# gwenzhang/GGA

Measured on AMD Instinct MI355X. Metric: kitti_frames_per_sec_gga_train_step, higher is better.
Workload: dtype f32 tensors; products on 2 x f16 operand planes (block-scaled), f32 accumulate - measured no less accurate than fp32 kernels: per convolution 0.7 x (dense) / 0.7-1.2 x (sparse) the RMS error of an fp32 FMA chain vs float64, whole-step losses over 8 seeds <= 2.5e-5 from float64 (fp32 CPU step: <= 1.6

## Files before the change

gga_amd/_lib.py:

```python
import ctypes as C
import os
import subprocess

_HERE = os.path.dirname(os.path.abspath(__file__))
LIB_PATH = os.path.join(_HERE, 'libgga_hip.so')
ABI_VERSION = 35

_lib = None

vp, i32, i64, f32, sz = C.c_void_p, C.c_int, C.c_int64, C.c_float, C.c_size_t
I3 = C.POINTER(C.c_int32 * 3)


class VoxelParams(C.Structure):
    _fields_ = [('voxel_size', C.c_float * 3), ('pc_range', C.c_float * 6),
                ('max_points', C.c_int32), ('max_voxels', C.c_int32)]


class PfnParams(C.Structure):
    _fields_ = [('voxel_size', C.c_float * 3), ('offsets', C.c_float * 3), ('eps', C.c_float),
                ('momentum', C.c_float), ('training', C.c_int32), ('in_features', C.c_int32),
                ('channels', C.c_int32)]


# ... 52 lines not shown
    'gga_hard_voxelize_workspace_bytes': (sz, [i32, i64]),
    'gga_hard_voxelize_batch': (i32, [vp, i32, C.POINTER(C.c_int64), i32, C.POINTER(VoxelParams),
                                       vp, vp, vp, vp, vp, sz, vp]),
    'gga_hard_voxelize_prepared': (i32, [vp, i32, C.POINTER(C.c_int64), vp, i32, C.POINTER(VoxelParams),
                                          vp, vp, vp, vp, vp, sz, vp]),
    'gga_dynamic_voxelize': (i32, [vp, i32, C.POINTER(C.c_int64), vp, i32, C.POINTER(VoxelParams), vp, vp, vp]),
    'gga_dynamic_voxel_map_workspace_bytes': (sz, [i64]),
    'gga_dynamic_voxel_map': (i32, [vp, vp, i32, i64, i32, i32, i32, i32, vp, vp, vp, vp, vp, vp, sz, vp]),
    'gga_dynamic_scatter_chunk': (i32, []),
    'gga_dynamic_scatter_workspace_bytes': (sz, [i64, i32]),
    'gga_dynamic_scatter_fwd': (i32, [vp, i32, i64, vp, vp, vp, vp, i64, i32, vp, vp, vp, sz, vp]),
    'gga_dynamic_scatter_bwd': (i32, [vp, i32, i64, vp, vp, vp, i64, i32, vp, vp]),
    'gga_dynamic_pfn_workspace_bytes': (sz, [i64]),
    'gga_dynamic_pfn_fwd': (i32, [vp, vp, i64, vp, vp, vp, vp, i64, C.POINTER(PfnParams)] + [vp] * 10 + [sz, vp]),
    'gga_dynamic_pfn_bwd': (i32, [vp, vp, i64, vp, i64, C.POINTER(PfnParams)] + [vp] * 11 + [sz, vp]),
    'gga_points_prepare_workspace_bytes': (sz, [i32, i64, i64]),
    'gga_points_prepare_batch': (i32, [vp, C.POINTER(C.c_int64), vp, C.POINTER(C.c_int64), vp, C.POINTER(C.c_int64),
                                        i32, i32, C.c_double, vp, C.POINTER(C.c_uint64), vp, vp, vp, sz, vp]),
    'gga_voxel_mean': (i32, [vp, vp, i64, i32, i32, i32, vp, vp]),
    'gga_pfn_workspace_bytes': (sz, [i64]),
    'gga_pfn_fwd': (i32, [vp, vp, vp, i64, vp, i32, C.POINTER(PfnParams), vp, vp, vp, vp, vp, vp, vp, vp, vp, sz, vp]),
    'gga_pfn_bwd': (i32, [vp, vp, vp, i64, vp, i32, C.POINTER(PfnParams), vp, vp, vp, vp, vp, vp, vp, vp, vp, vp, sz, vp]),
    'gga_pillar_scatter_map_bytes': (sz, [i32, i32, i32]),
    'gga_pillar_scatter_fwd': (i32, [vp, vp, i64, vp, i32, i32, i32, i32, i32, i32, vp, vp, vp]),
    'gga_pillar_scatter_bwd': (i32, [vp, vp, i64, vp, i32, i32, i32, i32, i32, vp, vp]),
    'gga_pillar_conv_map': (i32, [vp, i64, vp, i32, i32, i32, i32, i32, i32, i32, i32, i32, vp, vp]),
    'gga_sparse_index_bytes': (sz, [i64]),
    'gga_sparse_build_index': (i32, [vp, i64, i32, i32, i32, i32, vp, sz, vp]),
    'gga_sparse_out_index_bytes': (sz, [i64, i32]),
    'gga_sparse_out_sites_workspace_bytes': (sz, [i64, i32]),
    'gga_sparse_conv_out_sites': (i32, [vp, i64, i32, I3, I3, I3, I3, I3, vp, i64, vp, vp, sz, vp, sz, vp]),
    'gga_sparse_rulebook': (i32, [vp, i64, vp, i64, i32, I3, I3, I3, I3, I3, vp, i64, vp, i64, vp, vp, vp]),
    'gga_sparse_rowmask': (i32, [vp, i64, i32, vp, vp]),
    'gga_sparse_mask_order_workspace_bytes': (sz, [i64]),
    'gga_sparse_morton_order_workspace_bytes': (sz, [i64]),
    'gga_sparse_morton_order': (i32, [vp, i64, i32, i32, vp, vp, sz, vp]),
    'gga_sparse_mask_order': (i32, [vp, i64, i32, vp, vp, sz, vp]),
    'gga_sparse_split_weight_bytes': (sz, [i32, i32, i32]),
    'gga_sparse_conv_wgrad_workspace_bytes': (sz, [i64, i32, i32, i32]),
    'gga_dense_wgrad3x3_workspace_bytes': (sz, [i32, i32, i32, i32, i32]),
    'gga_sparse_pack_weight_planes': (i32, [vp, i32, i32, i32, i32, i32, vp, vp, vp]),
    'gga_sparse_conv_apply_stats': (i32, [vp, vp, vp, vp, vp, i64, i32, i32, i32, i32, vp, i64, i32, vp, vp, vp, vp]),
    'gga_sparse_conv_apply_tiles': (i64, [i64]),
    'gga_sparse_conv_apply_bn_bwd': (i32, [vp, vp, vp, vp, vp, i64, i32, i32, i32, i32, vp, i64, i32, vp, vp, vp, vp, i64, vp, vp, vp, vp, vp]),
    'gga_sparse_bev_nhwc_fwd': (i32, [vp, vp, i64, i32, i32, i32, i32, i32, vp, vp]),
    'gga_sparse_bev_nhwc_bwd': (i32, [vp, vp, i64, i32, i32, i32, i32, i32, vp, vp]),
    'gga_sparse_halo_tile_rows': (i64, []),
    'gga_sparse_halo_build': (i32, [vp, vp, i64, i64, i32, i32, vp, vp, vp, vp]),
    'gga_sparse_conv_apply_halo': (i32, [vp, vp, vp, vp, i32, vp, vp, i64, i64, i32, i32, i32, i32, vp, i64, i32, vp, vp, vp, vp, i64, vp, vp, vp, vp, vp]),
    'gga_sparse_conv_wgrad_planes': (i32, [vp, i64, vp, i64, vp, i64, i32, i32, i32, vp, i32, vp, vp, vp, sz, vp]),
    'gga_deconv_stream_tiles': (i64, [i64, i32, i32]),
    'gga_deconv_stream_fwd': (i32, [vp, vp, vp, vp, i32, i32, i32, i32, i32, i32, vp, vp, vp]),
    'gga_deconv_stream_bwd': (i32, [vp, vp, vp, vp, i32, i32, i32, i32, i32, i32, vp, vp]),
    'gga_absmax_bits': (i32, [vp, i64, i32, i64, vp, vp]),
    'gga_dense_conv3x3_pack_planes': (i32, [vp, i64, i64, i64, i64, i32, i32, i32, i32, vp, vp, vp]),
    'gga_dense_conv3x3_levels': (i32, [i32, vp, vp, vp, vp, i32, i32, i32, vp, i64, i32, vp, vp, vp, i32, i32, vp, vp]),
    'gga_dense_conv3x3_bn_bwd_pays': (i32, [i32, i32, i32, i32]),
    'gga_dense_conv3x3_bn_bwd_pays_planes': (i32, [i32, i32, i32, i32, i32]),
    'gga_dense_conv3x3_bn_bwd': (i32, [vp, vp, i32, i32, i32, i32, i32, vp, i64, i32, vp, i32, vp, vp, vp, i64, vp, vp, vp, vp, vp]),
    'gga_absmax_table_blocks': (i64, [i64]),
    'gga_absmax_table': (i32, [vp, i32, i64, vp, i32, vp]),
    'gga_pack_weights_table': (i32, [vp, i32, i64, i32, vp]),
    'gga_dense_wgrad3x3_block_amax': (i32, [vp, vp, i32, i32, i32, i32, i32, vp, i64, i64, i64, i64, i32, i32, vp, i32, vp, i32, vp, sz, vp]),
    'gga_dense_conv3x3_tile_rows': (i32, [i32, i32, i32, i32, i32]),
    'gga_dense_conv3x3_stat_rows': (i64, [i32, i32, i32, i32, i32, i32]),
    'gga_bn_relu_workspace_bytes': (sz, [i64, i32]),
    'gga_bn_relu_mask_bytes': (sz, [i64, i32]),
    'gga_bn_relu_fwd': (i32, [vp, vp, vp, vp, vp, vp, i64, i32, f32, f32, i32, i32, vp, i64, vp, vp, vp, i32, vp, vp, sz, vp]),
    'gga_bn_relu_bwd': (i32, [vp, i64, vp, vp, vp, vp, i64, i32, i32, i32, vp, vp, vp, vp, vp, vp, sz, vp]),
    'gga_column_sums': (i32, [vp, i64, i32, vp, vp, sz, vp]),
    'gga_bn_relu_bwd_partials': (i32, [vp, i64, vp, vp, vp, i64, i32, i32, vp, i32, vp, vp, vp, vp, vp, sz, vp]),
    'gga_gn_relu_workspace_bytes': (sz, [i32, i32]),
    'gga_gn_relu_fwd': (i32, [vp, vp, vp, i32, i64, i32, i32, f32, i32, vp, vp, vp, vp, vp, sz, vp]),
    'gga_gn_relu_bwd': (i32, [vp, vp, vp, vp, vp, i32, i64, i32, i32, i32, vp, vp, vp, vp, vp, sz, vp]),
    'gga_bn_stats': (i32, [vp, vp, vp, vp, vp, i64, i32, f32, f32, i32, vp, vp, vp, i32, i32, i32, vp, sz, vp]),
    'gga_head_conv3x3_fwd': (i32, [vp, i64, vp, vp, vp, i32, i32, i32, i32, i32, vp, vp]),
    'gga_head_conv3x3_fwd_tiles': (i32, [vp, i64, vp, vp, vp, i32, i32, i32, i32, i32, vp, vp, vp]),
    'gga_head_cell_tiles_count': (i64, [i32, i32, i32]),
    'gga_head_cell_tiles': (i32, [vp, i32, i32, i32, i32, vp, vp]),
    'gga_head_conv3x3_workspace_bytes': (sz, [i32]),
    'gga_head_conv3x3_wgrad': (i32, [vp, i64, vp, vp, i32, i32, i32, i32, i32, vp, vp, vp, sz, vp]),
    'gga_head_tail_bwd': (i32, [vp, vp, i64, vp, vp, vp, vp, i32, i32, i32, i32, i32, vp, i64, vp, vp, vp, vp, sz, vp]),
    'gga_head_tile_activity': (i32, [vp, i32, i32, i32, i32, vp, vp]),
    'gga_head_branch_bwd_workspace_bytes': (sz, [i32, i32, i32, i32]),
    'gga_head_branch_bwd': (i32, [vp, vp, i64, vp, vp, vp, vp, i32, i32, i32, i32, i32, vp, vp, vp, i64, vp, vp, vp, i32, vp, sz, vp]),
    'gga_heatmap_splat': (i32, [vp, i32, i32, i32, vp, i32, vp, vp, i32, vp]),
    'gga_focal_loss_workspace_bytes': (sz, [i64, i32]),
    'gga_focal_loss_fwd': (i32, [C.POINTER(TaskTable), f32, f32, f32, vp, sz, vp]),
    'gga_focal_loss_bwd': (i32, [C.POINTER(TaskTable), f32, f32, f32, vp]),
    'gga_gather_pred_fwd': (i32, [C.POINTER(TaskTable), i32, i32, i32, i32, vp]),
    'gga_gather_pred_bwd': (i32, [C.POINTER(TaskTable), i32, i32, i32, i32, vp]),
    'gga_box_losses_workspace_bytes': (sz, [i32, i32, i32]),
    'gga_box_losses_fwd': (i32, [C.POINTER(TaskTable), C.POINTER(LossParams), vp, sz, vp]),
    'gga_box_losses_bwd': (i32, [C.POINTER(TaskTable), i32, i32, vp]),
    'gga_box_iou_rotated': (i32, [vp, i32, vp, i32, i32, i32, vp, vp]),
    'gga_nms_rotated_workspace_bytes': (sz, [i32]),
    'gga_nms_rotated_sorted': (i32, [vp, i32, f32, i32, vp, vp, vp, sz, vp]),
    'gga_circle_nms_sorted': (i32, [vp, i32, C.c_double, i32, vp, vp, vp, sz, vp]),
    'gga_region_grow_workspace_bytes': (sz, [i64, i32]),
    'gga_region_grow': (i32, [vp, i64, i32, vp, vp, vp, i32, C.c_double, i32, vp, vp, sz, vp]),
    'gga_points_in_convex_polyhedra': (i32, [vp, i64, i32, vp, vp, i32, i32, vp, vp]),
    'gga_plane_inliers': (i32, [vp, i64, i32, vp, i32, C.c_double, vp, vp, vp]),
    'gga_image_box_match': (i32, [vp, vp, vp, vp, i32, i64, i32, vp, vp, vp, vp, vp]),
    'gga_kitti_eval_overlaps': (i32, [vp, vp, i64, vp, vp, i64, i32, i32, i32, i32, vp, vp, i64, vp]),
    'gga_kitti_eval_stats_workspace_bytes': (sz, [i32, i32, i32]),
    'gga_kitti_eval_stats': (i32, [vp, i32, vp, i64, vp, vp, vp, vp, i64, vp, i64, vp, i64, vp, vp, i32, vp, vp, i32, i32, i32, i32, i32,
# ... 69 lines not shown
```

gga_amd/pillar_conv.py:

```python
import torch
from torch import nn

from . import _lib
from . import functional as F
from ._lib import check


class PillarSupport:
    __slots__ = ('feats', 'coors', 'num_valid')

    def __init__(self, feats, coors, num_valid):
        self.feats, self.coors, self.num_valid = feats, coors, num_valid


def eligible(conv, canvas):
    sup = getattr(canvas, 'pillar_support', None)
    return (sup is not None and type(conv) is nn.Conv2d and conv.bias is None and conv.groups == 1
            and tuple(conv.dilation) == (1, 1) and conv.padding_mode == 'zeros' and not isinstance(conv.padding, str)
            and canvas.is_cuda and canvas.dtype == torch.float32 and torch.is_grad_enabled()
            and (sup.feats.requires_grad or conv.weight.requires_grad)
            and conv.in_channels <= 128 and conv.out_channels <= 128 and conv.in_channels % 4 == 0
            and canvas.is_contiguous(memory_format=torch.channels_last))


class _PillarConv2d(torch.autograd.Function):
    @staticmethod
    def forward(ctx, feats, weight, canvas, coors, num_valid, stride, padding):
        from . import strided_conv
        kh, kw = weight.shape[2:]
        if (strided_conv.ENABLED and kh == kw and stride[0] == stride[1] and padding[0] == padding[1] and stride[0] > 1
                and kh <= 5 and weight.shape[0] % 4 == 0):
            B, Ci, ny, nx = canvas.shape
            bk = strided_conv.book(B, ny, nx, kh, stride[0], padding[0], canvas.device)
            y, stats = strided_conv._apply(strided_conv._rows(canvas), bk.fwd, bk.fwd_mask, bk.fwd_perm,
                                           weight.detach().permute(2, 3, 1, 0).reshape(kh * kw, Ci, -1), bk.n_out,
                                           strided_conv._amax(feats.detach().contiguous()), want_stats=True)
            y = y.view(B, bk.Ho, bk.Wo, -1).permute(0, 3, 1, 2)
        else:
            y = torch.conv2d(canvas, weight, None, stride, padding)
            stats = torch.empty(0, dtype=torch.float64, device=y.device)
        ctx.save_for_backward(feats, weight, coors, num_valid)
        ctx.geom = (tuple(canvas.shape), stride, padding)
        ctx.mark_non_differentiable(stats)
        ctx.set_materialize_grads(False)
        return y, stats

    @staticmethod
    def backward(ctx, gy, _gstats=None):
        from .sparse import _Rulebook, _conv_apply, _pack_weight, conv_wgrad
        feats, w, coors, num_valid = ctx.saved_tensors
        (B, Ci, ny, nx), (sh, sw), (ph, pw) = ctx.geom
        Co, _, kh, kw = w.shape
        kvol, m = kh * kw, feats.shape[0]
        gy = gy.contiguous(memory_format=torch.channels_last)
        rows = gy.permute(0, 2, 3, 1).reshape(-1, Co)
        feats = feats.contiguous()
        L = _lib.lib()
        nbr = torch.empty((kvol, m), dtype=torch.int32, device=gy.device)
        check(L.gga_pillar_conv_map(F._p(coors), m, F._p(num_valid), B, ny, nx, kh, kw, sh, sw, ph, pw, F._p(nbr),
                                    F._stream()), 'gga_pillar_conv_map')
        gx = gw = None
        if ctx.needs_input_grad[0]:
            rb = _Rulebook(nbr)
            wk = w.permute(2, 3, 0, 1).reshape(kvol, Co, Ci).contiguous()
            gx = torch.empty_like(feats)
            _conv_apply(rows, rb, _pack_weight(wk, kvol, Co, Ci, 0), m, kvol, Co, Ci, 0, gx)
        if ctx.needs_input_grad[1]:
            g = torch.empty((kvol, Co, Ci), dtype=torch.float32, device=gy.device)
            conv_wgrad(rows, feats, nbr, m, kvol, Co, Ci, g)
            gw = g.view(kh, kw, Co, Ci).permute(2, 3, 0, 1)
        return gx, gw, None, None, None, None, None


def pillar_conv2d(canvas, conv):
    sup = canvas.pillar_support
    coors = sup.coors if sup.coors.dtype == torch.int32 else sup.coors.int()
    y, stats = _PillarConv2d.apply(sup.feats, conv.weight, canvas.detach(), coors.contiguous(), sup.num_valid,
                                   tuple(conv.stride), tuple(conv.padding))
    if stats.numel():
        F.attach_bn_partials(y, stats)
    return y
```

gga_amd/strided_conv.py:

```python
import ctypes as C
import os

import torch
from torch import nn

from . import _lib
from . import functional as F
from ._lib import check

ENABLED = True
STREAM = os.environ.get('GGA_DECONV_STREAM', '1') != '0'
STREAM_OFF = set()
_BOOKS = {}


class _Book:

    def __init__(self, B, H, W, k, s, p, device):
        Ho, Wo = (H + 2 * p - k) // s + 1, (W + 2 * p - k) // s + 1
        self.Ho, self.Wo, self.kvol = Ho, Wo, k * k
        self.n_in, self.n_out = B * H * W, B * Ho * Wo
        self._geom = (B, H, W, k, s, p, device)

    def __getattr__(self, name):
        side = name.split('_')[0]
        if side not in ('fwd', 'bwd') or name not in (side, side + '_mask', side + '_perm'):
            raise AttributeError(name)
        with torch.no_grad():
            m = self._map(side)
            mask, perm = self._order(m)
        self.__dict__.update({side: m, side + '_mask': mask, side + '_perm': perm})
        return self.__dict__[name]

    def _map(self, side):
        B, H, W, k, s, p, device = self._geom
        Ho, Wo = self.Ho, self.Wo
        b = torch.arange(B, device=device).view(B, 1, 1)
        oy, ox = torch.arange(Ho, device=device).view(1, Ho, 1), torch.arange(Wo, device=device).view(1, 1, Wo)
        iy_, ix_ = torch.arange(H, device=device).view(1, H, 1), torch.arange(W, device=device).view(1, 1, W)
        rows = []
        for ky in range(k):
            for kx in range(k):
                if side == 'fwd':
                    iy, ix = oy * s + ky - p, ox * s + kx - p
                    ok = (iy >= 0) & (iy < H) & (ix >= 0) & (ix < W)
                    rows.append(torch.where(ok, b * (H * W) + iy * W + ix, -1).reshape(-1))
                else:
                    ny, nx = iy_ + p - ky, ix_ + p - kx
                    ok = (ny >= 0) & (nx >= 0) & (ny % s == 0) & (nx % s == 0) & (ny // s < Ho) & (nx // s < Wo)
                    rows.append(torch.where(ok, b * (Ho * Wo) + (ny // s) * Wo + nx // s, -1).reshape(-1))
        return torch.stack(rows).int().contiguous()

    @staticmethod
    def _order(m):
        kvol, n = m.shape
        if kvol > 32:
            return None, None
        mask = torch.empty(n, dtype=torch.int32, device=m.device)
        check(_lib.lib().gga_sparse_rowmask(F._p(m), n, kvol, F._p(mask), F._stream()), 'gga_sparse_rowmask')
        if bool((mask == mask[0]).all()):
            return mask, None
        from .sparse import mask_order
        return mask, mask_order(mask, kvol)


# ... 32 lines not shown
            from . import dense_conv
            if dense_conv.RANGE_GUARD.armed:
                dense_conv.RANGE_GUARD.record(w_kio.detach())
    else:
        x_amax = w_amax = None
    y = torch.empty((n_rows, cout), dtype=torch.float32, device=x_rows.device)
    tiles = int(L.gga_sparse_conv_apply_tiles(n_rows)) if want_stats else 0
    parts = []
    for c0 in range(0, cout, 128):
        c1 = min(c0 + 128, cout)
        if bank:
            from . import weight_bank
            wp, w_amax = weight_bank.gather_operand(w_kio, planes, c0, c1)
        else:
            wp = torch.empty(L.gga_sparse_split_weight_bytes(kvol, cin, c1 - c0) // 2, dtype=torch.int16, device=y.device)
            check(L.gga_sparse_pack_weight_planes(F._p(w_kio[:, :, c0:c1].contiguous()), kvol, cin, c1 - c0, 0, planes, F._p(w_amax),
                                                  F._p(wp), F._stream()), 'gga_sparse_pack_weight_planes')
        st = torch.empty((tiles, 2, c1 - c0), dtype=torch.float64, device=y.device) if want_stats else None
        check(L.gga_sparse_conv_apply_stats(F._p(x_rows), F._p(m), F._p(wp), F._p(perm), F._p(mask), n_rows, kvol, cin,
                                            c1 - c0, 0, y.data_ptr() + 4 * c0, cout, planes, F._p(x_amax), F._p(w_amax),
                                            F._p(st), F._stream()), 'gga_sparse_conv_apply_stats')
        if want_stats:
            parts.append(st)
    if want_stats:
        return y, (parts[0] if len(parts) == 1 else torch.cat(parts, dim=2))
    return y


def _wgrad(x_rows, g_rows, m, n_rows, x_amax=None, g_amax=None):
    planes = _planes()
    if planes == 2:
        x_amax = _amax(x_rows) if x_amax is None else x_amax
        g_amax = _amax(g_rows) if g_amax is None else g_amax
    else:
        x_amax = g_amax = None
    L = _lib.lib()
    kvol, cin, cout = m.shape[0], x_rows.shape[1], g_rows.shape[1]
    gw = torch.empty((kvol, cin, cout), dtype=torch.float32, device=x_rows.device)
    for i0 in range(0, cin, 128):
        i1 = min(i0 + 128, cin)
        for o0 in range(0, cout, 128):
            o1 = min(o0 + 128, cout)
            whole = i1 - i0 == cin and o1 - o0 == cout
            part = gw if whole else torch.empty((kvol, i1 - i0, o1 - o0), dtype=torch.float32, device=gw.device)
            ws = F._workspace('sp_wgrad', L.gga_sparse_conv_wgrad_workspace_bytes(n_rows, kvol, i1 - i0, o1 - o0), gw.device)
            check(L.gga_sparse_conv_wgrad_planes(x_rows.data_ptr() + 4 * i0, cin, g_rows.data_ptr() + 4 * o0, cout, F._p(m),
                                                 n_rows, kvol, i1 - i0, o1 - o0, F._p(part), planes, F._p(x_amax), F._p(g_amax),
                                                 F._p(ws), ws.numel(), F._stream()), 'gga_sparse_conv_wgrad_planes')
            if not whole:
                gw[:, i0:i1, o0:o1] = part
    return gw


class _StridedConv(torch.autograd.Function):

    @staticmethod
    def forward(ctx, x, weight, k, s, p):
        B, cin, H, W = x.shape
        bk = book(B, H, W, k, s, p, x.device)
        w = weight.detach()
        x_amax = _amax(x)
        y, stats = _apply(_rows(x), bk.fwd, bk.fwd_mask, bk.fwd_perm, w.permute(2, 3, 1, 0), bk.n_out, x_amax, want_stats=True, bank=True)
        ctx.save_for_backward(x, weight)
        ctx.geom, ctx.amax = (k, s, p), (x_amax, None)
        ctx.mark_non_differentiable(stats)
        ctx.set_materialize_grads(False)
        return y.view(B, bk.Ho, bk.Wo, -1).permute(0, 3, 1, 2), stats

    @staticmethod
    def backward(ctx, gy, _gstats=None):
        x, weight = ctx.saved_tensors
        k, s, p = ctx.geom
        B, cin, H, W = x.shape
        cout = weight.shape[0]
        bk = book(B, H, W, k, s, p, x.device)
        gy = gy.contiguous(memory_format=torch.channels_last)
        g_rows = _rows(gy)
        gx = gw = None
        x_amax, w_amax = ctx.amax if _planes() == 2 else (None, None)
        g_amax = _amax(gy)
        if ctx.needs_input_grad[0]:
            w = weight.detach()
            gx = _apply(g_rows, bk.bwd, bk.bwd_mask, bk.bwd_perm, w.permute(2, 3, 0, 1), bk.n_in, g_amax, bank=True)
            gx = gx.view(B, H, W, cin).permute(0, 3, 1, 2)
        if ctx.needs_input_grad[1]:
            gw = _wgrad(_rows(x), g_rows, bk.fwd, bk.n_out, x_amax, g_amax).view(k, k, cin, cout).permute(3, 2, 0, 1)
        return gx, gw, None, None, None


def _stream_form(cin, cout, s, backward):
    if not STREAM or _planes() != 2 or cin not in (64, 128, 256) or cout % 128 or not 1 <= s <= 4:
        return False
    form = (s, 'bwd' if backward else 'fwd')
    return form not in STREAM_OFF and (not backward or cout in (128, 256, 512))


def _block_pointers(ops):
    return (C.c_void_p * len(ops))(*[op.data_ptr() for op in ops])


def _stream_fwd(x, weight, s, x_amax, want_stats=True):
    from . import dense_conv, weight_bank
    L = _lib.lib()
    B, cin, H, W = x.shape
    cout = weight.shape[1]
    w_kio = weight.detach().permute(2, 3, 0, 1)
    if dense_conv.RANGE_GUARD.armed:
        dense_conv.RANGE_GUARD.record(w_kio)
    ops = [weight_bank.gather_operand(w_kio, 2, c0, c0 + 128) for c0 in range(0, cout, 128)]
    x_amax = _amax(x) if x_amax is None else x_amax
    y = torch.empty((B, H * s, W * s, cout), dtype=torch.float32, device=x.device)
    tiles = int(L.gga_deconv_stream_tiles(B * H * W, cin, s))
    stats = torch.empty((tiles, 2, cout), dtype=torch.float64, device=x.device) if want_stats else None
    check(L.gga_deconv_stream_fwd(F._p(_rows(x)), _block_pointers([op for op, _ in ops]), F._p(x_amax), F._p(ops[0][1]), B, H, W,
                                  cin, cout, s, F._p(y), F._p(stats), F._stream()), 'gga_deconv_stream_fwd')
# ... 93 lines not shown
```

include/gga_hip.h:

```cpp
#ifndef GGA_HIP_H_
#define GGA_HIP_H_

#include <stddef.h>
#include <stdint.h>

#ifdef __cplusplus
extern "C" {
#endif

typedef enum {
    GGA_OK = 0,
    GGA_ERR_INVALID_ARG = -1,
    GGA_ERR_WORKSPACE = -2,
    GGA_ERR_LAUNCH = -3
} gga_status;

const char* gga_last_error(void);
int gga_abi_version(void);

enum {
    GGA_TIME_SCATTER_FWD = 0,
    GGA_TIME_DENSE_CONV = 1,
    GGA_TIME_SPARSE_CONV = 2,
    GGA_TIME_SPARSE_WGRAD = 3,
// ... 140 lines not shown
int64_t gga_dense_conv3x3_stat_rows(int B, int H, int W, int cout, int planes, int n_slices);
int gga_dense_conv3x3_tile_rows(int B, int H, int W, int cout, int planes);

int gga_absmax_bits(const float* x, int64_t rows, int width, int64_t row_stride, uint32_t* out_bits, void* stream);
typedef struct {
    const float* src;
    uint16_t* dst;
    const uint32_t* amax;
    int64_t s_k0, s_k1, s_c, s_col;
    int64_t first;
    int32_t kw, kvol, n_c, n_col, c0, col0, n_in, co, layout, reverse;
} GgaPackEntry;
typedef struct {
    const float* src;
    uint32_t* slot;
    int64_t n;
    int64_t first_block;
} GgaAmaxEntry;
int64_t gga_absmax_table_blocks(int64_t n);
int gga_absmax_table(const GgaAmaxEntry* table_device, int n_entries, int64_t n_blocks, uint32_t* slots, int n_slots, void* stream);
int gga_pack_weights_table(const GgaPackEntry* table_device, int n_entries, int64_t total, int planes, void* stream);
int gga_sparse_pack_weight_planes(const float* weight, int kvol, int cin, int cout, int transpose, int planes,
                                  const uint32_t* amax_weight, void* packed, void* stream);
int64_t gga_sparse_conv_apply_tiles(int64_t n_rows);
int gga_sparse_conv_apply_stats(const float* x, const int32_t* map, const void* split_weight, const int32_t* perm,
                                const uint32_t* rowmask, int64_t n_rows, int kvol, int cin, int cout, int flip, float* y,
                                int64_t y_row_stride, int planes, const uint32_t* amax_x, const uint32_t* amax_weight,
                                double* stats, void* stream);
int gga_sparse_conv_apply_bn_bwd(const float* x, const int32_t* map, const void* split_weight, const int32_t* perm,
                                 const uint32_t* rowmask, int64_t n_rows, int kvol, int cin, int cout, int flip, float* y,
                                 int64_t y_row_stride, int planes, const uint32_t* amax_x, const uint32_t* amax_weight,
                                 double* stats, const float* bn_x, int64_t bn_x_row_stride, const float* bn_gamma,
                                 const float* bn_beta, const float* bn_mean, const float* bn_invstd, void* stream);
int64_t gga_sparse_halo_tile_rows(void);
int gga_sparse_halo_build(const int32_t* nbr, const int32_t* tile_rows, int64_t n_rows, int64_t n_tiles, int kvol,
                          int halo_capacity, int32_t* halo_rows, int32_t* halo_counts, uint16_t* local_map, void* stream);
int gga_sparse_conv_apply_halo(const float* x, const void* split_weight, const int32_t* tile_rows,
                               const int32_t* halo_counts, int halo_capacity, const int32_t* halo_rows,
                               const uint16_t* local_map, int64_t n_rows, int64_t n_tiles, int kvol, int cin, int cout, int flip,
                               float* y, int64_t y_row_stride, int planes, const uint32_t* amax_x, const uint32_t* amax_weight,
                               double* stats, const float* bn_x, int64_t bn_x_row_stride, const float* bn_gamma,
                               const float* bn_beta, const float* bn_mean, const float* bn_invstd, void* stream);
size_t gga_sparse_conv_wgrad_workspace_bytes(int64_t n_rows, int kvol, int cin, int cout);
int gga_sparse_conv_wgrad_planes(const float* x, int64_t x_row_stride, const float* grad_out, int64_t grad_out_row_stride,
                                 const int32_t* nbr, int64_t n_rows, int kvol, int cin, int cout, float* grad_weight,
                                 int planes, const uint32_t* amax_x, const uint32_t* amax_grad_out, void* workspace,
                                 size_t workspace_bytes, void* stream);
int64_t gga_deconv_stream_tiles(int64_t n_pixels, int cin, int s);
int gga_deconv_stream_fwd(const float* x, const void* const* weight_blocks, const uint32_t* amax_x,
                          const uint32_t* amax_weight, int B, int h, int w, int cin, int cout, int s, float* y, double* stats,
                          void* stream);
int gga_deconv_stream_bwd(const float* gy, const void* const* weight_blocks, const uint32_t* amax_gy,
                          const uint32_t* amax_weight, int B, int h, int w, int cin, int cout, int s, float* gx, void* stream);
int gga_dense_conv3x3_pack_planes(const float* weight, int64_t stride_co, int64_t stride_ci, int64_t stride_ky,
                                  int64_t stride_kx, int cin, int cout, int backward, int planes,
                                  const uint32_t* amax_weight, void* packed, void* stream);
int gga_dense_conv3x3_bn_bwd_pays_planes(int B, int H, int W, int cout, int planes);
int gga_dense_conv3x3_bn_bwd_pays(int B, int H, int W, int cout);
int gga_dense_conv3x3_bn_bwd(const float* x, const void* split_weight, int B, int H, int W, int cin, int cout, float* y,
                             int64_t y_pixel_stride, int transposed, double* stats, int planes, const uint32_t* amax_x,
                             const uint32_t* amax_weight, const float* bn_x, int64_t bn_x_pixel_stride, const float* bn_gamma,
                             const float* bn_beta, const float* bn_mean, const float* bn_invstd, void* stream);
int gga_dense_conv3x3_levels(int n_entries, const float* const* x, const int32_t* heights, const int32_t* widths,
                             const void* const* split_weight, int B, int cin, int cout, float* const* y, int64_t y_pixel_stride,
                             int planes, const uint32_t* const* amax_x, const uint32_t* amax_weight, const float* const* bias,
                             int tile_rows, int transposed, double* const* stats, void* stream);
size_t gga_dense_wgrad3x3_workspace_bytes(int B, int H, int W, int cin, int cout);
int gga_dense_wgrad3x3_block_amax(const float* x, const float* grad_y, int B, int H, int W, int cin, int cout,
                                  float* grad_weight, int64_t stride_co, int64_t stride_ci, int64_t stride_ky,
                                  int64_t stride_kx, int transposed, int planes, const uint32_t* amax_x, int amax_x_per_block,
                                  const uint32_t* amax_grad_y, int amax_grad_y_per_block, void* workspace,
                                  size_t workspace_bytes, void* stream);

size_t gga_bn_relu_workspace_bytes(int64_t rows, int channels);
size_t gga_bn_relu_mask_bytes(int64_t rows, int channels);
int gga_bn_stats(const float* x, const float* gamma, const float* beta, float* running_mean, float* running_var,
                 int64_t rows, int channels, float eps, float momentum, int training, float* saved,
                 float* scale_shift, const double* partials, int n_partials, int partials_width, int column_offset,
                 void* workspace, size_t workspace_bytes, void* stream);
int gga_bn_relu_fwd(const float* x, const float* residual, const float* gamma, const float* beta,
                    float* running_mean, float* running_var, int64_t rows, int channels, float eps, float momentum,
                    int training, int relu, float* y, int64_t y_row_stride, void* mask_bits, float* saved,
                    const double* partials, int n_partials, uint32_t* amax_y, void* workspace, size_t workspace_bytes,
                    void* stream);
int gga_bn_relu_bwd(const float* grad_y, int64_t grad_y_row_stride, const float* x, const void* mask_bits,
                    const float* gamma, const float* saved, int64_t rows, int channels, int relu, int training, float* grad_x,
                    float* grad_residual, float* grad_gamma, float* grad_beta, uint32_t* amax_grad_x, void* workspace,
                    size_t workspace_bytes, void* stream);
int gga_column_sums(const float* x, int64_t rows, int channels, float* sums, void* workspace, size_t workspace_bytes,
                    void* stream);
int gga_bn_relu_bwd_partials(const float* grad_masked, int64_t grad_row_stride, const float* x, const float* gamma,
                             const float* saved, int64_t rows, int channels, int training, const double* partials,
                             int n_partials, float* grad_x, float* grad_gamma, float* grad_beta, uint32_t* amax_grad_x,
                             void* workspace, size_t workspace_bytes, void* stream);

size_t gga_gn_relu_workspace_bytes(int B, int channels);
int gga_gn_relu_fwd(const float* x, const float* gamma, const float* beta, int B, int64_t rows_per_sample, int channels,
                    int groups, float eps, int relu, float* y, float* stat, float* scale_shift, uint32_t* amax_y,
                    void* workspace, size_t workspace_bytes, void* stream);
int gga_gn_relu_bwd(const float* grad_y, const float* x, const float* gamma, const float* stat, const float* scale_shift,
                    int B, int64_t rows_per_sample, int channels, int groups, int relu, float* grad_x, float* grad_gamma,
                    float* grad_beta, uint32_t* amax_grad_x, void* workspace, size_t workspace_bytes, void* stream);

int gga_head_conv3x3_fwd(const float* x, int64_t x_pixel_stride, const float* in_scale_shift, const float* weight,
                         const float* bias, int B, int H, int W, int cin, int cout, float* y, void* stream);
int gga_head_conv3x3_fwd_tiles(const float* x, int64_t x_pixel_stride, const float* in_scale_shift, const float* weight,
// ... 213 lines not shown
```

tools_dev/deconv_stream_calls.py:

```python
import collections
import csv
import glob
import os
import re
import sys

FLOOR = 5.5e12
B, H, W = 16, 248, 216
N1, N2, N3 = B * H * W, B * H * W // 4, B * H * W // 16
LAYERS = {'D1': (N1, 64, N1, 128), 'D2': (N2, 128, N1, 128), 'D3': (N3, 256, N1, 128),
          'opener1': (4 * N1, 64, N1, 64), 'opener2': (N1, 64, N2, 128), 'opener3': (N2, 128, N3, 256)}


def last_step(d):
    f = max(glob.glob(os.path.join(d, '**', '*kernel_trace.csv'), recursive=True), key=os.path.getmtime)
    rows = list(csv.DictReader(open(f)))
    rows.sort(key=lambda r: int(r['Start_Timestamp']))
    opt = [i for i, r in enumerate(rows) if 'multi_tensor_apply' in r['Kernel_Name']]
    ends = [opt[i] for i in range(len(opt)) if i + 1 == len(opt) or opt[i + 1] - opt[i] > 50]
    return rows[ends[-3] + 1:ends[-1] + 1]


def us(r):
    return (int(r['End_Timestamp']) - int(r['Start_Timestamp'])) / 1e3


def short(name):
    return re.sub(r'^void ', '', name.split('(')[0])[:52]


def label(calls):
    out, seen = [], collections.Counter()
    fwd_order = ['opener1', 'opener2', 'opener3', 'opener3', 'D1', 'D2', 'D3']
    wgrad_order = ['D3', 'D3', 'D2', 'D1', 'opener3', 'opener3', 'opener2']
    n_fwd = 0
    for r in calls:
        name, wg = r['Kernel_Name'], int(r['Workgroup_Size_X'])
        tiles = int(r['Grid_Size_X']) // wg
        m = re.search(r'deconv_stream_(fwd|bwd)_kernel<([0-9, ]+)>', name)
        if 'NP = 3' in name or re.search(r', 3>', name):
            out.append(('pillars', 'weight gradient' if 'wgrad' in name else 'backward-data'))
        elif m and m.group(1) == 'fwd':
            out.append(({6696: 'D1', 1674: 'D2', 837: 'D3'}.get(tiles, '?'), 'forward'))
        elif m:
            out.append(({'1, 1, 64': 'D1', '1, 2, 128': 'D2', '2, 2, 128': 'D3'}.get(m.group(2), '?'), 'backward-data'))
        elif 'wgrad' in name:
            out.append((wgrad_order[seen['w']] if seen['w'] < len(wgrad_order) else '?', 'weight gradient'))
            seen['w'] += 1
        elif seen['w'] == 0 and n_fwd < len(fwd_order):
            out.append((fwd_order[n_fwd], 'forward'))
            n_fwd += 1
        else:
            have = {l for l, d in out if d == 'backward-data'}
            neck, opener = {419: ('D3', 'D3'), 1674: ('D2', 'opener3'), 6696: ('D1', 'opener2')}.get(tiles, ('?', '?'))
            out.append((neck if neck not in have or tiles == 419 else opener, 'backward-data'))
    return out


def need_bytes(layer, direction, half=False):
    if layer not in LAYERS or direction == 'weight gradient':
        return None
    n_in, cin, n_out, cout = LAYERS[layer]
    d = 2 if half else 1
    return 4 * (n_in * cin // d + n_out * cout) if direction == 'backward-data' else 4 * (n_in * cin + n_out * cout // d)


def main():
    step = last_step(sys.argv[1])
    pat = re.compile(r'sp_conv_x9_kernel|sp_conv_wgrad_x9_kernel|deconv_stream_')
    calls = [r for r in step if pat.search(r['Kernel_Name'])]
    print(f'{"us":>8}  {"tiles":>6}  {"layer":8} {"direction":15} {"need MB":>8} {"TB/s":>6} {"of floor":>8}  kernel')
    for r, (layer, direction) in zip(calls, label(calls)):
        t = us(r)
        half = 'sp_conv_x9' in r['Kernel_Name'] and ((layer == 'D3' and direction == 'backward-data') or (layer == 'opener3' and direction == 'forward'))
        nb = need_bytes(layer, direction, half)
        rate = f'{nb / t / 1e6:6.2f} {nb / FLOOR / (t * 1e-6):8.2f}' if nb else f'{"":6} {"":8}'
        mb = f'{nb / 1e6:8.0f}' if nb else f'{"":8}'
        print(f'{t:8.1f}  {int(r["Grid_Size_X"]) // int(r["Workgroup_Size_X"]):6d}  {layer:8} {direction:15} {mb} {rate}  {short(r["Kernel_Name"])}')
    tot = collections.defaultdict(float)
    for r in step:
        tot[short(r['Kernel_Name'])] += us(r)
    other = collections.defaultdict(float)
    two = len(sys.argv) > 2
    if two:
        for r in last_step(sys.argv[2]):
            other[short(r['Kernel_Name'])] += us(r)
    print(f'\nstep: {sum(tot.values()) / 1e3:.3f} ms busy in {len(step)} launches' + (f'; other trace {sum(other.values()) / 1e3:.3f} ms' if two else ''))
    for k in sorted(set(tot) | set(other), key=lambda k: -max(tot[k], other[k])):
        if max(tot[k], other[k]) >= 20 or abs(tot[k] - other[k]) >= 30:
            print(f'{tot[k] / 1e3:9.3f} ms' + (f' {other[k] / 1e3:9.3f} ms {(tot[k] - other[k]) / 1e3:+8.3f}' if two else '') + f'  {k}')


if __name__ == '__main__':
    main()
```

Before: 538.4.

## Add streaming dense kernel for stride-2 3x3 conv forward

Adds a dedicated HIP kernel for stride-2, 3x3, pad-1 convolution forward. It computes output pixel coordinates directly for interior tiles instead of going through the gather rulebook, stages input rows in LDS as two fp16 planes, and shares the overlapping kx=2 column with the neighbouring output pixel. The kernel also emits per-tile BN statistics. Strided forward calls in the pillar and generic paths are routed through it, except the 128->256 shape, which stays on the old path. This trades the generic sparse gather for specialised code with several template variants and adds another kernel to maintain.

```diff
diff --git a/gga_amd/_lib.py b/gga_amd/_lib.py
--- a/gga_amd/_lib.py
+++ b/gga_amd/_lib.py
@@ -128,6 +128,8 @@
     'gga_deconv_stream_tiles': (i64, [i64, i32, i32]),
     'gga_deconv_stream_fwd': (i32, [vp, vp, vp, vp, i32, i32, i32, i32, i32, i32, vp, vp, vp]),
     'gga_deconv_stream_bwd': (i32, [vp, vp, vp, vp, i32, i32, i32, i32, i32, i32, vp, vp]),
+    'gga_strided_stream_tiles': (i64, [i64]),
+    'gga_strided_stream_fwd': (i32, [vp, vp, vp, vp, vp, i32, i32, i32, i32, i32, i32, vp, vp, vp]),
     'gga_absmax_bits': (i32, [vp, i64, i32, i64, vp, vp]),
     'gga_dense_conv3x3_pack_planes': (i32, [vp, i64, i64, i64, i64, i32, i32, i32, i32, vp, vp, vp]),
     'gga_dense_conv3x3_levels': (i32, [i32, vp, vp, vp, vp, i32, i32, i32, vp, i64, i32, vp, vp, vp, i32, i32, vp, vp]),
diff --git a/gga_amd/csrc/strided_stream.hip b/gga_amd/csrc/strided_stream.hip
--- /dev/null
+++ b/gga_amd/csrc/strided_stream.hip
@@ -0,0 +1,274 @@
+#include "gga_common.h"
+#include "conv_planes.h"
+
+#define SS_THREADS 256
+#define SS_TILE 128
+
+typedef uint32_t ss_u4 __attribute__((ext_vector_type(4)));
+union SsFrag { ss_u4 q; mf_v8h v; };
+
+static inline int ss_sb(int cin, int cout) { return cin == 64 && cout <= 128 ? 64 : 32; }
+static inline size_t ss_lds(int cin, int cout) {
+    return (size_t)3 * ss_sb(cin, cout) * (4 * cin + 16) + SS_TILE * (sizeof(int64_t) + 2 * sizeof(int)) + (size_t)8 * cout * sizeof(float);
+}
+
+template <int CH, int SB, int CT, int WC>
+__global__ __launch_bounds__(SS_THREADS, 2) void strided_stream_fwd_kernel(const float* __restrict__ X, const uint16_t* __restrict__ Wp0,
+                                                                         const uint16_t* __restrict__ Wp1, const int32_t* __restrict__ perm,
+                                                                         float* __restrict__ Y, double* __restrict__ stats,
+                                                                         const uint32_t* __restrict__ amax_x,
+                                                                         const uint32_t* __restrict__ amax_w, int64_t n_rows,
+                                                                         int64_t n_border, int H, int W, int cout) {
+    constexpr int cin = 32 * CH;
+    constexpr int co = WC == 2 ? 64 : 128;
+    constexpr int NB = CT == 1 ? 3 : 2;
+    constexpr int NRB = SB / 32;
+    constexpr int RBW = NRB * WC / 4;
+    static_assert(RBW >= 1, "more waves across the rows than row blocks");
+    constexpr int C4S = CH == 2 ? 4 : 5;
+    constexpr int RSTEP = SS_THREADS >> C4S;
+    constexpr int RPT = SB / RSTEP;
+    constexpr int rowb = 4 * cin + 16;
+    constexpr int NST = 9 * CH;
+    extern __shared__ __attribute__((aligned(16))) unsigned char ss_smem[];
+    unsigned char* const Xs = ss_smem;
+    int64_t* const ibase = reinterpret_cast<int64_t*>(ss_smem + 3 * SB * rowb);
+    int* const pixs = reinterpret_cast<int*>(ibase + SS_TILE);
+    int* const flags = pixs + SS_TILE;
+    float* const red = reinterpret_cast<float*>(flags + SS_TILE);
+    const int tid = threadIdx.x, lane = tid & 63, wave = tid >> 6;
+    const int r = lane & 31, hh = lane >> 5;
+    const int Ho = H >> 1, Wo = W >> 1;
+    const int sbx = h2_scale_exp(*amax_x), sbw = h2_scale_exp(*amax_w);
+    const float xscale = h2_scale(sbx);
+    const int64_t tile = blockIdx.x;
+    const int64_t q0 = tile * SS_TILE;
+
+    int my_ox = 0, my_pix = -1;
+    if (tid < SS_TILE) {
+        const int64_t q = q0 + tid;
+        if (q < n_rows) {
+            if (q0 >= n_border) {
+                const int Wi = Wo - 1, Hi = Ho - 1;
+                const int64_t j = q - n_border;
+                const int64_t b = j / ((int64_t)Hi * Wi);
+                const int rem = (int)(j - b * Hi * Wi);
+                const int oy = 1 + rem / Wi;
+                my_pix = (int)((b * Ho + oy) * Wo + 1 + (rem - (oy - 1) * Wi));
+            } else {
+                my_pix = perm[q];
+            }
+            if (my_pix < 0 || my_pix >= n_rows) my_pix = -1;
+        }
+        int64_t ib = 0;
+        int fl = 0;
+        if (my_pix >= 0) {
+            const int b = my_pix / (Ho * Wo);
+            const int rem = my_pix - b * Ho * Wo;
+            const int oy = rem / Wo;
+            my_ox = rem - oy * Wo;
+            ib = (((int64_t)b * H + 2 * oy - 1) * W + 2 * my_ox - 1) * cin;
+            fl = 8 | (oy == 0 ? 1 : 0) | (my_ox == 0 ? 2 : 0);
+        }
+        pixs[tid] = my_pix;
+        ibase[tid] = ib;
+        flags[tid] = fl;
+    }
+    __syncthreads();
+    if (tid < SS_TILE && (tid & (SB - 1)) != SB - 1 && my_pix >= 0 && my_ox != Wo - 1 && pixs[tid + 1] == my_pix + 1) flags[tid] |= 4;
+    __syncthreads();
+
+    const int ct0 = (wave % WC) * CT, rb0 = (wave / WC) * RBW;
+    const uint16_t* wl[CT];
+    int qsw[CT], gcol[CT];
+#pragma unroll
+    for (int j = 0; j < CT; ++j) {
+        gcol[j] = (ct0 + j) * 32 + r;
+        const int c = gcol[j] % co;
+        wl[j] = (gcol[j] / co ? Wp1 : Wp0) + c * 32;
+        qsw[j] = (c >> 2) & 3;
+    }
+    auto load_b = [&](int st, SsFrag (&b)[CT][2][2]) {
+#pragma unroll
+        for (int j = 0; j < CT; ++j) {
+            const uint16_t* src = wl[j] + (int64_t)st * (2 * co * 32);
+#pragma unroll
+            for (int ks = 0; ks < 2; ++ks)
+#pragma unroll
+                for (int p = 0; p < 2; ++p)
+                    b[j][ks][p].q = *reinterpret_cast<const ss_u4*>(src + p * (co * 32) + (((2 * ks + hh) ^ qsw[j]) << 3));
+        }
+    };
+    const float dx = h2_descale(sbx), dw = h2_descale(sbw);
+    mf_v16 acc[CT][RBW], total[CT][RBW];
+#pragma unroll
+    for (int j = 0; j < CT; ++j)
+#pragma unroll
+        for (int rb = 0; rb < RBW; ++rb)
+#pragma unroll
+            for (int i = 0; i < 16; ++i) { acc[j][rb][i] = 0.0f; total[j][rb][i] = 0.0f; }
+    SsFrag bq[NB][CT][2][2];
+    load_b(0, bq[0]);
+    if (NB == 3) load_b(1, bq[1]);
+    const int piece = tid & ((1 << C4S) - 1), lrow = tid >> C4S;
+
+    for (int sb = 0; sb < SS_TILE / SB; ++sb) {
+        if (q0 + sb * SB >= n_rows) break;
+        const unsigned char* xrow[RBW];
+#pragma unroll
+        for (int rb = 0; rb < RBW; ++rb) {
+            const int L = (rb0 + rb) * 32 + r;
+            xrow[rb] = Xs + ((flags[sb * SB + L] & 4) ? L + 1 : 2 * SB + L) * rowb + hh * 16;
+        }
+        int64_t sbase[RPT];
+        int sfl[RPT];
+#pragma unroll
+        for (int j = 0; j < RPT; ++j) {
+            const int i = sb * SB + lrow + RSTEP * j;
+            sbase[j] = ibase[i] + 4 * piece;
+            sfl[j] = flags[i];
+        }
+        for (int ky = 0; ky < 3; ++ky) {
+            {
+                float4 v[3][RPT];
+                bool ok[2][RPT];
+                const int64_t koff = (int64_t)ky * W * cin;
+#pragma unroll
+                for (int j = 0; j < RPT; ++j) {
+                    ok[1][j] = (sfl[j] & 8) && !(ky == 0 && (sfl[j] & 1));
+                    ok[0][j] = ok[1][j] && !(sfl[j] & 2);
+                    v[0][j] = *reinterpret_cast<const float4*>(X + (ok[0][j] ? sbase[j] + koff : 4 * piece));
+                    v[1][j] = *reinterpret_cast<const float4*>(X + (ok[1][j] ? sbase[j] + koff + cin : 4 * piece));
+                }
+#pragma unroll
+                for (int j = 0; j < RPT; ++j)
+                    if (!(sfl[j] & 4)) v[2][j] = *reinterpret_cast<const float4*>(X + (ok[1][j] ? sbase[j] + koff + 2 * cin : 4 * piece));
+                auto put = [&](const float4& f, bool valid, int slot) {
+                    const float sc = valid ? xscale : 0.0f;
+                    uint2 p0, p1;
+                    h2_split2s(f.x, f.y, sc, p0.x, p1.x);
+                    h2_split2s(f.z, f.w, sc, p0.y, p1.y);
+                    unsigned char* dst = Xs + slot * rowb + 8 * piece;
+                    *reinterpret_cast<uint2*>(dst) = p0;
+                    *reinterpret_cast<uint2*>(dst + 2 * cin) = p1;
+                };
+#pragma unroll
+                for (int j = 0; j < RPT; ++j) {
+                    const int L = lrow + RSTEP * j;
+                    put(v[0][j], ok[0][j], L);
+                    put(v[1][j], ok[1][j], SB + L);
+                    if (!(sfl[j] & 4)) put(v[2][j], ok[1][j], 2 * SB + L);
+                }
+            }
+            __syncthreads();
+#pragma unroll
+            for (int s = 0; s < 3 * CH; ++s) {
+                const int kx = s / CH, ch = s % CH;
+                int nxt = ky * 3 * CH + s + NB - 1;
+                nxt = nxt >= NST ? nxt - NST : nxt;
+                load_b(nxt, bq[(s + NB - 1) % NB]);
+                __builtin_amdgcn_sched_barrier(0);
+                SsFrag (&bc)[CT][2][2] = bq[s % NB];
+#pragma unroll
+                for (int ks = 0; ks < 2; ++ks) {
+                    SsFrag a[RBW][2];
+#pragma unroll
+                    for (int rb = 0; rb < RBW; ++rb) {
+                        const unsigned char* arow = kx == 2 ? xrow[rb] : Xs + (kx * SB + (rb0 + rb) * 32 + r) * rowb + hh * 16;
+#pragma unroll
+                        for (int p = 0; p < 2; ++p)
+                            a[rb][p].q = *reinterpret_cast<const ss_u4*>(arow + p * 2 * cin + ch * 64 + ks * 32);
+                    }
+#define SS_MH(PA, PB) _Pragma("unroll") for (int j = 0; j < CT; ++j) _Pragma("unroll") for (int rb = 0; rb < RBW; ++rb) acc[j][rb] = __builtin_amdgcn_mfma_f32_32x32x16_f16(a[rb][PA].v, bc[j][ks][PB].v, acc[j][rb], 0, 0, 0);
+                    SS_MH(0, 1) SS_MH(1, 0) SS_MH(0, 0)
+#undef SS_MH
+                }
+                if (ch == CH - 1) {
+#pragma unroll
+                    for (int j = 0; j < CT; ++j)
+#pragma unroll
+                        for (int rb = 0; rb < RBW; ++rb) {
+                            total[j][rb] += acc[j][rb];
+#pragma unroll
+                            for (int i = 0; i < 16; ++i) acc[j][rb][i] = 0.0f;
+                        }
+                }
+            }
+            __syncthreads();
+        }
+#pragma unroll
+        for (int j = 0; j < CT; ++j)
+#pragma unroll
+            for (int rb = 0; rb < RBW; ++rb) {
+                float s1 = 0.0f, s2 = 0.0f;
+#pragma unroll
+                for (int v = 0; v < 16; ++v) {
+                    const int pix = pixs[sb * SB + (rb0 + rb) * 32 + (v >> 2) * 8 + hh * 4 + (v & 3)];
+                    const float val = (total[j][rb][v] + 0.0f) * dx * dw;
+                    total[j][rb][v] = 0.0f;
+                    if (pix >= 0) Y[(int64_t)pix * cout + gcol[j]] = val;
+                    s1 += val; s2 = fmaf(val, val, s2);
+                }
+                s1 += __shfl_xor(s1, 32);
+                s2 += __shfl_xor(s2, 32);
+                if (hh == 0) {
+                    const int blk = sb * NRB + rb0 + rb;
+                    red[(blk * 2 + 0) * cout + gcol[j]] = s1;
+                    red[(blk * 2 + 1) * cout + gcol[j]] = s2;
+                }
+            }
+    }
+    if (!stats) return;
+    const int done = (int)((n_rows - q0 + SB - 1) / SB) * NRB;
+    __syncthreads();
+    for (int i = tid; i < 2 * cout; i += SS_THREADS) {
+        const int which = i / cout, c = i - which * cout;
+        double a = 0.0;
+#pragma unroll
+        for (int w_ = 0; w_ < 4; ++w_) a += w_ < done ? (double)red[(w_ * 2 + which) * cout + c] : 0.0;
+        stats[(tile * 2 + which) * cout + c] = a;
+    }
+}
+
+extern "C" int64_t gga_strided_stream_tiles(int64_t n_out_pixels) { return n_out_pixels < 1 ? 0 : (n_out_pixels + SS_TILE - 1) / SS_TILE; }
+
+extern "C" int gga_strided_stream_fwd(const float* x, const void* const* weight_blocks, const int32_t* perm, const uint32_t* amax_x,
+                                      const uint32_t* amax_weight, int B, int H, int W, int cin, int cout, int planes, float* y,
+                                      double* stats, void* stream_) {
+    hipStream_t stream = (hipStream_t)stream_;
+    const char* who = "gga_strided_stream_fwd";
+    GGA_REQUIRE(x && weight_blocks && perm && amax_x && amax_weight && y, "%s: null pointer argument", who);
+    GGA_REQUIRE(planes == 2, "%s: planes %d (two fp16 planes only)", who, planes);
+    GGA_REQUIRE(cin == 64 || cin == 128, "%s: cin %d is not 64 or 128", who, cin);
+    GGA_REQUIRE(cout == 128 || cout == 256 || (cout == 64 && cin == 64), "%s: cout %d is not 128 or 256 (or 64 with cin 64)", who, cout);
+    GGA_REQUIRE(B >= 1 && H >= 2 && W >= 2, "%s: bad sizes (B=%d H=%d W=%d)", who, B, H, W);
+    GGA_REQUIRE(H % 2 == 0 && W % 2 == 0, "%s: odd map size %d x %d", who, H, W);
+    GGA_REQUIRE((int64_t)B * H * W < ((int64_t)1 << 31), "%s: %lld input rows (B * H * W must stay below 2^31)", who, (long long)B * H * W);
+    const int nblocks = cout == 256 ? 2 : 1;
+    for (int c = 0; c < nblocks; ++c) GGA_REQUIRE(weight_blocks[c], "%s: null pointer argument (weight block %d)", who, c);
+    const int Ho = H / 2, Wo = W / 2;
+    const int64_t n_rows = (int64_t)B * Ho * Wo, n_border = (int64_t)B * (Ho + Wo - 1);
+    const int64_t n_tiles = gga_strided_stream_tiles(n_rows);
+    const size_t lds = ss_lds(cin, cout);
+    static bool once = false;
+    if (!once) {
+        GGA_CHECK_HIP(hipFuncSetAttribute((const void*)strided_stream_fwd_kernel<2, 64, 1, 2>, hipFuncAttributeMaxDynamicSharedMemorySize, 64 * 1024), "strided_stream_fwd_kernel: LDS size");
+        GGA_CHECK_HIP(hipFuncSetAttribute((const void*)strided_stream_fwd_kernel<2, 64, 1, 4>, hipFuncAttributeMaxDynamicSharedMemorySize, 64 * 1024), "strided_stream_fwd_kernel: LDS size");
+        GGA_CHECK_HIP(hipFuncSetAttribute((const void*)strided_stream_fwd_kernel<4, 32, 1, 4>, hipFuncAttributeMaxDynamicSharedMemorySize, 64 * 1024), "strided_stream_fwd_kernel: LDS size");
+        GGA_CHECK_HIP(hipFuncSetAttribute((const void*)strided_stream_fwd_kernel<4, 32, 2, 4>, hipFuncAttributeMaxDynamicSharedMemorySize, 64 * 1024), "strided_stream_fwd_kernel: LDS size");
+        GGA_CHECK_HIP(hipFuncSetAttribute((const void*)strided_stream_fwd_kernel<2, 32, 2, 4>, hipFuncAttributeMaxDynamicSharedMemorySize, 64 * 1024), "strided_stream_fwd_kernel: LDS size");
+        once = true;
+    }
+    const uint16_t* w0 = (const uint16_t*)weight_blocks[0];
+    const uint16_t* w1 = nblocks == 2 ? (const uint16_t*)weight_blocks[1] : w0;
+    const dim3 grid((unsigned)n_tiles), block(SS_THREADS);
+#define SS_LAUNCH(CH, SB, CT, WC) hipLaunchKernelGGL((strided_stream_fwd_kernel<CH, SB, CT, WC>), grid, block, lds, stream, x, w0, w1, perm, y, stats, amax_x, amax_weight, n_rows, n_border, H, W, cout)
+    if (cin == 128 && cout == 256) SS_LAUNCH(4, 32, 2, 4);
+    else if (cin == 128) SS_LAUNCH(4, 32, 1, 4);
+    else if (cout == 256) SS_LAUNCH(2, 32, 2, 4);
+    else if (cout == 128) SS_LAUNCH(2, 64, 1, 4);
+    else SS_LAUNCH(2, 64, 1, 2);
+#undef SS_LAUNCH
+    GGA_CHECK_LAUNCH("strided_stream_fwd_kernel");
+    return GGA_OK;
+}
diff --git a/gga_amd/pillar_conv.py b/gga_amd/pillar_conv.py
--- a/gga_amd/pillar_conv.py
+++ b/gga_amd/pillar_conv.py
@@ -32,9 +32,9 @@
                 and kh <= 5 and weight.shape[0] % 4 == 0):
             B, Ci, ny, nx = canvas.shape
             bk = strided_conv.book(B, ny, nx, kh, stride[0], padding[0], canvas.device)
-            y, stats = strided_conv._apply(strided_conv._rows(canvas), bk.fwd, bk.fwd_mask, bk.fwd_perm,
-                                           weight.detach().permute(2, 3, 1, 0).reshape(kh * kw, Ci, -1), bk.n_out,
-                                           strided_conv._amax(feats.detach().contiguous()), want_stats=True)
+            y, stats = strided_conv.conv_fwd_rows(strided_conv._rows(canvas), bk, (B, ny, nx, kh, stride[0], padding[0]),
+                                                  weight.detach().permute(2, 3, 1, 0),
+                                                  strided_conv._amax(feats.detach().contiguous()), bank=False)
             y = y.view(B, bk.Ho, bk.Wo, -1).permute(0, 3, 1, 2)
         else:
             y = torch.conv2d(canvas, weight, None, stride, padding)
diff --git a/gga_amd/strided_conv.py b/gga_amd/strided_conv.py
--- a/gga_amd/strided_conv.py
+++ b/gga_amd/strided_conv.py
@@ -11,6 +11,8 @@
 ENABLED = True
 STREAM = os.environ.get('GGA_DECONV_STREAM', '1') != '0'
 STREAM_OFF = set()
+STRIDED_STREAM = os.environ.get('GGA_STRIDED_STREAM', '1') != '0'
+STRIDED_STREAM_OFF = set() if os.environ.get('GGA_STRIDED_STREAM') == 'all' else {((128, 256), 'fwd')}
 _BOOKS = {}
 
 
@@ -149,6 +151,51 @@
     return gw
 
 
+def _strided_stream_form(cin, cout, k, s, p, H, W, backward=False):
+    if not STRIDED_STREAM or _planes() != 2 or backward or (k, s, p) != (3, 2, 1) or H % 2 or W % 2 or H < 2 or W < 2:
+        return False
+    if cin not in (64, 128) or not (cout in (128, 256) or (cin, cout) == (64, 64)):
+        return False
+    return ((cin, cout), 'fwd') not in STRIDED_STREAM_OFF
+
+
+def _strided_stream_fwd(x_rows, bk, B, H, W, w_kio, x_amax, bank):
+    from . import dense_conv, weight_bank
+    L = _lib.lib()
+    w_kio = w_kio.detach()
+    cin, cout = w_kio.shape[-2:]
+    x_amax = _amax(x_rows) if x_amax is None else x_amax
+    if bank:
+        if dense_conv.RANGE_GUARD.armed:
+            dense_conv.RANGE_GUARD.record(w_kio)
+        ops = [weight_bank.gather_operand(w_kio, 2, c0, min(c0 + 128, cout)) for c0 in range(0, cout, 128)]
+        wps, w_amax = [op for op, _ in ops], ops[0][1]
+    else:
+        w9 = w_kio.reshape(9, cin, cout)
+        w_amax, wps = _amax(w9), []
+        for c0 in range(0, cout, 128):
+            c1 = min(c0 + 128, cout)
+            wp = torch.empty(L.gga_sparse_split_weight_bytes(9, cin, c1 - c0) // 2, dtype=torch.int16, device=x_rows.device)
+            check(L.gga_sparse_pack_weight_planes(F._p(w9[:, :, c0:c1].contiguous()), 9, cin, c1 - c0, 0, 2, F._p(w_amax), F._p(wp),
+                                                  F._stream()), 'gga_sparse_pack_weight_planes')
+            wps.append(wp)
+    y = torch.empty((bk.n_out, cout), dtype=torch.float32, device=x_rows.device)
+    stats = torch.empty((int(L.gga_strided_stream_tiles(bk.n_out)), 2, cout), dtype=torch.float64, device=y.device)
+    check(L.gga_strided_stream_fwd(F._p(x_rows), _block_pointers(wps), F._p(bk.fwd_perm), F._p(x_amax), F._p(w_amax), B, H, W, cin, cout,
+                                   2, F._p(y), F._p(stats), F._stream()), 'gga_strided_stream_fwd')
+    return y, stats
+
+
+def conv_fwd_rows(x_rows, bk, geom, w_kio, x_amax, bank):
+    B, H, W, k, s, p = geom
+    cin, cout = w_kio.shape[-2:]
+    if _strided_stream_form(cin, cout, k, s, p, H, W):
+        return _strided_stream_fwd(x_rows, bk, B, H, W, w_kio, x_amax, bank)
+    if not bank:
+        w_kio = w_kio.reshape(k * k, cin, cout)
+    return _apply(x_rows, bk.fwd, bk.fwd_mask, bk.fwd_perm, w_kio, bk.n_out, x_amax, want_stats=True, bank=bank)
+
+
 class _StridedConv(torch.autograd.Function):
 
     @staticmethod
@@ -157,7 +204,7 @@
         bk = book(B, H, W, k, s, p, x.device)
         w = weight.detach()
         x_amax = _amax(x)
-        y, stats = _apply(_rows(x), bk.fwd, bk.fwd_mask, bk.fwd_perm, w.permute(2, 3, 1, 0), bk.n_out, x_amax, want_stats=True, bank=True)
+        y, stats = conv_fwd_rows(_rows(x), bk, (B, H, W, k, s, p), w.permute(2, 3, 1, 0), x_amax, bank=True)
         ctx.save_for_backward(x, weight)
         ctx.geom, ctx.amax = (k, s, p), (x_amax, None)
         ctx.mark_non_differentiable(stats)
diff --git a/include/gga_hip.h b/include/gga_hip.h
--- a/include/gga_hip.h
+++ b/include/gga_hip.h
@@ -216,6 +216,10 @@
                           void* stream);
 int gga_deconv_stream_bwd(const float* gy, const void* const* weight_blocks, const uint32_t* amax_gy,
                           const uint32_t* amax_weight, int B, int h, int w, int cin, int cout, int s, float* gx, void* stream);
+int64_t gga_strided_stream_tiles(int64_t n_out_pixels);
+int gga_strided_stream_fwd(const float* x, const void* const* weight_blocks, const int32_t* perm, const uint32_t* amax_x,
+                           const uint32_t* amax_weight, int B, int H, int W, int cin, int cout, int planes, float* y,
+                           double* stats, void* stream);
 int gga_dense_conv3x3_pack_planes(const float* weight, int64_t stride_co, int64_t stride_ci, int64_t stride_ky,
                                   int64_t stride_kx, int cin, int cout, int backward, int planes,
                                   const uint32_t* amax_weight, void* packed, void* stream);
diff --git a/tools_dev/deconv_stream_calls.py b/tools_dev/deconv_stream_calls.py
--- a/tools_dev/deconv_stream_calls.py
+++ b/tools_dev/deconv_stream_calls.py
@@ -38,7 +38,12 @@
         name, wg = r['Kernel_Name'], int(r['Workgroup_Size_X'])
         tiles = int(r['Grid_Size_X']) // wg
         m = re.search(r'deconv_stream_(fwd|bwd)_kernel<([0-9, ]+)>', name)
-        if 'NP = 3' in name or re.search(r', 3>', name):
+        ms = re.search(r'strided_stream_fwd_kernel', name)
+        if ms:
+            layer = {6696: 'opener1', 1674: 'opener2', 419: 'opener3'}.get(tiles, '?')
+            out.append((layer, 'forward'))
+            n_fwd += 2 if layer == 'opener3' else 1
+        elif 'NP = 3' in name or re.search(r', 3>', name):
             out.append(('pillars', 'weight gradient' if 'wgrad' in name else 'backward-data'))
         elif m and m.group(1) == 'fwd':
             out.append(({6696: 'D1', 1674: 'D2', 837: 'D3'}.get(tiles, '?'), 'forward'))
@@ -67,7 +72,7 @@
 
 def main():
     step = last_step(sys.argv[1])
-    pat = re.compile(r'sp_conv_x9_kernel|sp_conv_wgrad_x9_kernel|deconv_stream_')
+    pat = re.compile(r'sp_conv_x9_kernel|sp_conv_wgrad_x9_kernel|deconv_stream_|strided_stream_')
     calls = [r for r in step if pat.search(r['Kernel_Name'])]
     print(f'{"us":>8}  {"tiles":>6}  {"layer":8} {"direction":15} {"need MB":>8} {"TB/s":>6} {"of floor":>8}  kernel')
     for r, (layer, direction) in zip(calls, label(calls)):
```

Result: no change. 538.7, median of 4 (+0.1%).
